# jmschrei/blueberry

Measured on AMD Instinct MI355X. Metric: Gpair-updates/s per stress iteration, N=50k, higher is better.
Workload: dtype f32

## Files before the change

blueberry_amd/csrc/bb_solver_kernels.h:

```cpp
#pragma once

#include "bb_solver_device.h"

namespace {

__device__ __forceinline__ void rsqrt_sqrt_f64(double d2, double &rinv, double &dist) {
    const double r0 = __builtin_amdgcn_rsq(d2);
    const double t = d2 * r0;
    const double e = fma(-t, r0, 1.0);
    const double q = e * fma(e, 0.375, 0.5);
    rinv = fma(r0, q, r0);
    dist = fma(t, q, t);
}
__device__ __forceinline__ double weight01_f64(double delta) {
    return __builtin_fmin(__builtin_fmax(delta * 0x1p1000, 0.0), 1.0);
}

__device__ __forceinline__ double rcp_f64(double x) {
    const double r0 = __builtin_amdgcn_rcp(x);
    const double e = fma(-x, r0, 1.0);
    return fma(r0, fma(e, e, e), r0);
}

template <int C, int OP>
__device__ __forceinline__ void pair_step(const double2 &drow, double xi, double yi, double zi,
                                          const double (&xj)[2][3], double (&gc)[2][3], double &gx,
                                          double &gy, double &gz, double &s) {
    using T = double;
    const T delta = C == 0 ? drow.x : drow.y;
    if constexpr (OP == kOpMatvec2) {
        const T a = delta * delta;
        gx += a * xj[C][0]; gy += a * xj[C][1]; gz += a * xj[C][2];
        gc[C][0] += a * xi; gc[C][1] += a * yi; gc[C][2] += a * zi;
        return;
    }
    const T dx = xi - xj[C][0], dy = yi - xj[C][1], dz = zi - xj[C][2];
    const T d2 = fma(dx, dx, fma(dy, dy, fma(dz, dz, Traits<T>::eps2())));
    T rinv, dist;
    rsqrt_sqrt_f64(d2, rinv, dist);
    if constexpr (is_weighted_op<OP>()) {
        const T m = weight01_f64(delta);
        const T res = fma(dist, m, -delta);
        const T r = rcp_f64(delta + (1.0 - m));
        const T u = res * r;
        T coef;
        if constexpr (OP == kOpStressW1) {
            s = fma(res, u, s);
            coef = u * rinv;
        } else {
            s = fma(u, u, s);
            coef = (u * r) * rinv;
        }
        gx = fma(coef, dx, gx); gy = fma(coef, dy, gy); gz = fma(coef, dz, gz);
        gc[C][0] = fma(-coef, dx, gc[C][0]);
        gc[C][1] = fma(-coef, dy, gc[C][1]);
        gc[C][2] = fma(-coef, dz, gc[C][2]);
        return;
    }
    const T res = fma(dist, weight01_f64(delta), -delta);
    s = fma(res, res, s);
    const T coef = res * rinv;
    gx = fma(coef, dx, gx); gy = fma(coef, dy, gy); gz = fma(coef, dz, gz);
    gc[C][0] = fma(-coef, dx, gc[C][0]);
    gc[C][1] = fma(-coef, dy, gc[C][1]);
    gc[C][2] = fma(-coef, dz, gc[C][2]);
}

typedef float f32x4_raw __attribute__((ext_vector_type(4)));
typedef double f64x2_raw __attribute__((ext_vector_type(2)));
template <bool NT>
__device__ __forceinline__ float4 stream_load(const float4 *p) {
    if constexpr (NT) {
        const f32x4_raw v = __builtin_nontemporal_load(reinterpret_cast<const f32x4_raw *>(p));
        return make_float4(v.x, v.y, v.z, v.w);
    } else {
        return *p;
    }
}
template <bool NT>
__device__ __forceinline__ double2 stream_load(const double2 *p) {
    if constexpr (NT) {
        const f64x2_raw v = __builtin_nontemporal_load(reinterpret_cast<const f64x2_raw *>(p));
        return make_double2(v.x, v.y);
    } else {
        return *p;
    }
}

template <typename Vec>
struct WinPtr {
    const Vec *p;
    template <bool NT>
    __device__ __forceinline__ Vec load(int k) const { return stream_load<NT>(p + k * 64); }
};

template <bool NT, int OP, typename XR, typename WIN>
__device__ __forceinline__ void process_unit_f64n(double2 (&d)[8], const XR &xrow, const WIN &next,
                                                  const double (&xj)[1][2][3], double (&gc)[1][2][3],
                                                  double &stress, __amdgpu_buffer_rsrc_t row_rsrc,
                                                  unsigned row_voff) {
    double s = 0.0;
#pragma unroll
    for (int r = 0; r < 8; ++r) {
        const double xi = xrow.get(3 * r), yi = xrow.get(3 * r + 1), zi = xrow.get(3 * r + 2);
        double gx = 0.0, gy = 0.0, gz = 0.0;
        pair_step<0, OP>(d[r], xi, yi, zi, xj[0], gc[0], gx, gy, gz, s);
        pair_step<1, OP>(d[r], xi, yi, zi, xj[0], gc[0], gx, gy, gz, s);
        d[r] = next.template load<NT>(r);
        wave_sum_hi3(gx, gy, gz);
        store_row3(row_rsrc, row_voff + r * 24u, gx, gy, gz);
        __builtin_amdgcn_sched_barrier(0);
    }
    stress += s;
}

typedef double f64x4 __attribute__((ext_vector_type(4)));

__device__ __forceinline__ double swap_sum16(double t) {
    const unsigned lo = (unsigned)__double2loint(t), hi = (unsigned)__double2hiint(t);
    const auto a = __builtin_amdgcn_permlane16_swap(lo, lo, false, false);
    const auto b = __builtin_amdgcn_permlane16_swap(hi, hi, false, false);
    return __hiloint2double((int)b[0], (int)a[0]) + __hiloint2double((int)b[1], (int)a[1]);
}
__device__ __forceinline__ double swap_sum32(double t) {
    const unsigned lo = (unsigned)__double2loint(t), hi = (unsigned)__double2hiint(t);
    const auto a = __builtin_amdgcn_permlane32_swap(lo, lo, false, false);
    const auto b = __builtin_amdgcn_permlane32_swap(hi, hi, false, false);
    return __hiloint2double((int)b[0], (int)a[0]) + __hiloint2double((int)b[1], (int)a[1]);
}

__device__ __forceinline__ float swap_add32(float a, float b) {
    const auto s = __builtin_amdgcn_permlane32_swap(__float_as_uint(a), __float_as_uint(b), false, false);
    return __uint_as_float(s[0]) + __uint_as_float(s[1]);
}
__device__ __forceinline__ float swap_add16(float a, float b) {
    const auto s = __builtin_amdgcn_permlane16_swap(__float_as_uint(a), __float_as_uint(b), false, false);
    return __uint_as_float(s[0]) + __uint_as_float(s[1]);
}
__device__ __forceinline__ float row16_sum3(float a, float b, float c) {
    float t, u, w;
    asm("s_nop 1\n\t"
        "v_add_f32_dpp %0, %3, %3 row_mirror row_mask:0xf bank_mask:0xf\n\t"
        "v_add_f32_dpp %0, %5, %5 row_mirror row_mask:0xf bank_mask:0xc\n\t"
        "v_add_f32_dpp %1, %4, %4 row_mirror row_mask:0xf bank_mask:0xf\n\t"
        "s_nop 0\n\t"
        "v_add_f32_dpp %2, %0, %0 row_half_mirror row_mask:0xf bank_mask:0xf\n\t"
        "v_add_f32_dpp %2, %1, %1 row_half_mirror row_mask:0xf bank_mask:0x2\n\t"
        "s_nop 1\n\t"
        "v_add_f32_dpp %2, %2, %2 quad_perm:[1,0,3,2] row_mask:0xf bank_mask:0xf\n\t"
        "s_nop 1\n\t"
        "v_add_f32_dpp %2, %2, %2 quad_perm:[2,3,0,1] row_mask:0xf bank_mask:0xf"
        : "=&v"(t), "=v"(u), "=v"(w)
        : "v"(a), "v"(b), "v"(c));
    return w;
}
template <int R>
__device__ __forceinline__ void row_sums_step(const float (&g)[12], float (&h)[6], float (&m)[3]) {
    if constexpr (R == 0) h[0] = swap_add32(g[0], g[1]);
    if constexpr (R == 1) {
        h[1] = swap_add32(g[2], g[3]); h[2] = swap_add32(g[4], g[5]);
        m[0] = swap_add16(h[0], h[1]);
    }
    if constexpr (R == 2) { h[3] = swap_add32(g[6], g[7]); m[1] = swap_add16(h[2], h[3]); }
    if constexpr (R == 3) {
        h[4] = swap_add32(g[8], g[9]); h[5] = swap_add32(g[10], g[11]);
        m[2] = swap_add16(h[4], h[5]);
    }
}
__device__ __forceinline__ int swap_rowsum_slot(int lane) {
    const int row = lane >> 4, bank = (lane >> 2) & 3;
    return 4 * (bank < 3 ? bank : 2) + ((row & 1) << 1) + (row >> 1);
}
__device__ __forceinline__ bool swap_rowsum_stores(int lane) { return (lane & 3) == 0 && (lane & 12) != 12; }

template <bool NT, int OP, typename XR, typename WIN>
__device__ __forceinline__ void process_unit_f64w(double2 (&d)[8], const XR &xrow,
                                                  const WIN &next,
                                                  const double (&xj)[4][2][3], double (&gc)[4][2][3],
                                                  const double (&sel)[6], double &stress,
                                                  __amdgpu_buffer_rsrc_t row_rsrc, unsigned row_voff,
                                                  int stage_idx) {
    extern __shared__ __attribute__((aligned(16))) float row_lds[];
    double s = 0.0;
    f64x4 acc = {0.0, 0.0, 0.0, 0.0};
#pragma unroll
    for (int r = 0; r < 2; ++r) {
        const double xi = xrow.get(3 * r), yi = xrow.get(3 * r + 1), zi = xrow.get(3 * r + 2);
        double gx = 0.0, gy = 0.0, gz = 0.0;
#pragma unroll
        for (int k = 0; k < 4; ++k) {
            pair_step<0, OP>(d[r * 4 + k], xi, yi, zi, xj[k], gc[k], gx, gy, gz, s);
            pair_step<1, OP>(d[r * 4 + k], xi, yi, zi, xj[k], gc[k], gx, gy, gz, s);
            d[r * 4 + k] = next.template load<NT>(r * 4 + k);
        }
        acc = __builtin_amdgcn_mfma_f64_16x16x4f64(gx, sel[3 * r + 0], acc, 0, 0, 0);
        acc = __builtin_amdgcn_mfma_f64_16x16x4f64(gy, sel[3 * r + 1], acc, 0, 0, 0);
        acc = __builtin_amdgcn_mfma_f64_16x16x4f64(gz, sel[3 * r + 2], acc, 0, 0, 0);
    }
    double t = (acc.x + acc.y) + (acc.z + acc.w);
    t = swap_sum16(t);
    t = swap_sum32(t);
    *reinterpret_cast<double *>(row_lds + stage_idx) = t;
    const u32x2 bits = {(unsigned)__double2loint(t), (unsigned)__double2hiint(t)};
    __builtin_amdgcn_raw_buffer_store_b64(bits, row_rsrc, row_voff, 0, 0);
    stress += s;
}

typedef float f32x2 __attribute__((ext_vector_type(2)));

struct StripF32 {
    f32x2 x[2][2][3];
    f32x2 g[2][2][3];
};

__device__ __forceinline__ f32x2 weight01(f32x2 delta) {
    f32x2 w;
    const f32x2 big = {0x1p100f, 0x1p100f};
    asm("v_pk_mul_f32 %0, %1, %2 clamp" : "=v"(w) : "v"(delta), "v"(big));
    return w;
}

template <int K, int H, bool FIRST, int OP, bool MASK = true>
__device__ __forceinline__ void pair_step2(f32x2 delta, f32x2 xi, f32x2 yi, f32x2 zi, StripF32 &st,
                                           f32x2 &rx, f32x2 &ry, f32x2 &rz, f32x2 &s2) {
    static_assert(MASK || OP == kOpStress, "only the plain stress sweep has a mask-free form");
    if constexpr (OP == kOpMatvec2) {
        const f32x2 a = delta * delta;
        if constexpr (FIRST) {
            rx = a * st.x[K][H][0]; ry = a * st.x[K][H][1]; rz = a * st.x[K][H][2];
        } else {
            rx += a * st.x[K][H][0]; ry += a * st.x[K][H][1]; rz += a * st.x[K][H][2];
        }
        st.g[K][H][0] += a * xi;
        st.g[K][H][1] += a * yi;
        st.g[K][H][2] += a * zi;
        return;
    }
    const f32x2 eps2 = {1e-30f, 1e-30f};
    const f32x2 dx = xi - st.x[K][H][0], dy = yi - st.x[K][H][1], dz = zi - st.x[K][H][2];
    const f32x2 d2 = dx * dx + (dy * dy + (dz * dz + eps2));
    f32x2 rinv;
    rinv.x = __builtin_amdgcn_rsqf(d2.x);
    rinv.y = __builtin_amdgcn_rsqf(d2.y);
    if constexpr (is_weighted_op<OP>()) {
        const f32x2 res = (d2 * rinv - delta) * weight01(delta);
        f32x2 a = delta;
        if constexpr (OP == kOpStressW2) a = delta * delta;
        f32x2 w;
        w.x = __builtin_amdgcn_rcpf(__builtin_fmaxf(a.x, 0x1p-126f));
        w.y = __builtin_amdgcn_rcpf(__builtin_fmaxf(a.y, 0x1p-126f));
        const f32x2 t = res * w;
        s2 += res * t;
        const f32x2 coef = t * rinv;
        if constexpr (FIRST) {
            rx = coef * dx; ry = coef * dy; rz = coef * dz;
        } else {
            rx += coef * dx; ry += coef * dy; rz += coef * dz;
        }
        st.g[K][H][0] -= coef * dx;
        st.g[K][H][1] -= coef * dy;
        st.g[K][H][2] -= coef * dz;
        return;
    }
    f32x2 res = d2 * rinv - delta;
    if constexpr (MASK) res *= weight01(delta);
    s2 += res * res;
    const f32x2 coef = res * rinv;
    if constexpr (FIRST) {
        rx = coef * dx; ry = coef * dy; rz = coef * dz;
    } else {
        rx += coef * dx; ry += coef * dy; rz += coef * dz;
    }
    st.g[K][H][0] -= coef * dx;
    st.g[K][H][1] -= coef * dy;
    st.g[K][H][2] -= coef * dz;
}

template <bool ROW3>
__device__ __forceinline__ void pk24_decode(float &word, unsigned base) {
    if constexpr (ROW3) {
        asm volatile("v_add_u32 %0, %0, %1" : "+v"(word) : "s"(base));
    } else {
        asm volatile("v_mad_u32_u24 %0, %0, 1, %1" : "+v"(word) : "s"(base));
    }
}
template <bool ROW3>
__device__ __forceinline__ void pk24_decode(float4 &w, unsigned base) {
    pk24_decode<ROW3>(w.x, base); pk24_decode<ROW3>(w.y, base);
    pk24_decode<ROW3>(w.z, base); pk24_decode<ROW3>(w.w, base);
}
__device__ __forceinline__ void pk24_decode_to(float &dst, float src, unsigned base) {
    asm volatile("v_mad_u32_u24 %0, %1, 1, %2" : "=v"(dst) : "v"(src), "s"(base));
}
__device__ __forceinline__ void pk24_decode_to(float4 &dst, const float4 &src, unsigned base) {
    pk24_decode_to(dst.x, src.x, base); pk24_decode_to(dst.y, src.y, base);
    pk24_decode_to(dst.z, src.z, base); pk24_decode_to(dst.w, src.w, base);
}
constexpr unsigned kPk24SelPair = 0x0c0c0703u;
constexpr unsigned kPk24SelThird = 0x0c070100u;
__device__ __forceinline__ float pk24_tops(float hi, float lo, unsigned sel) {
    float v;
    asm volatile("v_perm_b32 %0, %1, %2, %3" : "=v"(v) : "v"(hi), "v"(lo), "s"(sel));
    return v;
}
__device__ __forceinline__ float4 pk24_tops(float4 hi, float4 lo, unsigned sel) {
    return make_float4(pk24_tops(hi.x, lo.x, sel), pk24_tops(hi.y, lo.y, sel),
                       pk24_tops(hi.z, lo.z, sel), pk24_tops(hi.w, lo.w, sel));
}

template <bool NT, int OP, bool PK = false, typename WIN>
__device__ __forceinline__ void process_unit_f32(float4 (&d)[8], const float (&xrow)[12],
                                                 const WIN &next, StripF32 &st,
                                                 double &stress, __amdgpu_buffer_rsrc_t row_rsrc,
                                                 unsigned row_voff, int stage_idx,
                                                 unsigned base = 0u) {
    extern __shared__ __attribute__((aligned(16))) float row_lds[];
    f32x2 s2 = {0.f, 0.f};
    float g[12], h[6], m[3];
    auto row = [&](auto rc) __attribute__((always_inline)) {
        constexpr int r = decltype(rc)::value;
        const float xs = xrow[3 * r], ys = xrow[3 * r + 1], zs = xrow[3 * r + 2];
        const f32x2 xi = {xs, xs}, yi = {ys, ys}, zi = {zs, zs};
        f32x2 rx, ry, rz;
        if constexpr (PK) {
            constexpr int A = r < 3 ? 2 * r : 6, B = r == 0 ? 1 : (r == 1 ? 2 : (r == 2 ? 5 : 7));
            if constexpr (r == 0) d[6] = pk24_tops(d[1], d[0], kPk24SelPair);
            if constexpr (r == 1) d[6] = pk24_tops(d[2], d[6], kPk24SelThird);
            if constexpr (r == 2) {
                d[7] = pk24_tops(d[3], pk24_tops(d[5], d[4], kPk24SelPair), kPk24SelThird);
                d[3] = next.template load<NT>(3);
            }
            pk24_decode<r == 3>(d[A], base);
            pair_step2<0, 0, true, OP, false>(f32x2{d[A].x, d[A].y}, xi, yi, zi, st, rx, ry, rz, s2);
            pair_step2<0, 1, false, OP, false>(f32x2{d[A].z, d[A].w}, xi, yi, zi, st, rx, ry, rz, s2);
            if constexpr (r == 0) d[0] = next.template load<NT>(0);
            if constexpr (r == 2) d[4] = next.template load<NT>(4);
            if constexpr (r == 1) pk24_decode_to(d[2], d[3], base);
            else pk24_decode<r == 3>(d[B], base);
            pair_step2<1, 0, false, OP, false>(f32x2{d[B].x, d[B].y}, xi, yi, zi, st, rx, ry, rz, s2);
            pair_step2<1, 1, false, OP, false>(f32x2{d[B].z, d[B].w}, xi, yi, zi, st, rx, ry, rz, s2);
            if constexpr (r == 0) d[1] = next.template load<NT>(1);
            if constexpr (r == 1) d[2] = next.template load<NT>(2);
            if constexpr (r == 2) d[5] = next.template load<NT>(5);
            g[3 * r] = rx.x + rx.y; g[3 * r + 1] = ry.x + ry.y; g[3 * r + 2] = rz.x + rz.y;
            row_sums_step<r>(g, h, m);
            return;
        }
        pair_step2<0, 0, true, OP>(f32x2{d[2 * r].x, d[2 * r].y}, xi, yi, zi, st, rx, ry, rz, s2);
        pair_step2<0, 1, false, OP>(f32x2{d[2 * r].z, d[2 * r].w}, xi, yi, zi, st, rx, ry, rz, s2);
        d[2 * r] = next.template load<NT>(2 * r);
        pair_step2<1, 0, false, OP>(f32x2{d[2 * r + 1].x, d[2 * r + 1].y}, xi, yi, zi, st, rx, ry, rz, s2);
        pair_step2<1, 1, false, OP>(f32x2{d[2 * r + 1].z, d[2 * r + 1].w}, xi, yi, zi, st, rx, ry, rz, s2);
        d[2 * r + 1] = next.template load<NT>(2 * r + 1);
        g[3 * r] = rx.x + rx.y; g[3 * r + 1] = ry.x + ry.y; g[3 * r + 2] = rz.x + rz.y;
        row_sums_step<r>(g, h, m);
    };
    row(std::integral_constant<int, 0>{});
    row(std::integral_constant<int, 1>{});
    row(std::integral_constant<int, 2>{});
    row(std::integral_constant<int, 3>{});
    const float keep = row16_sum3(m[0], m[1], m[2]);
    row_lds[stage_idx] = keep;
    __builtin_amdgcn_raw_buffer_store_b32(__float_as_uint(keep), row_rsrc, row_voff, 0, 0);
    stress += (double)(s2.x + s2.y);
}

__device__ __forceinline__ void load_strip(StripF32 &st, const float *__restrict__ X, int j0,
                                           int lane) {
#pragma unroll
    for (int k = 0; k < 2; ++k) {
        const float4 *p = reinterpret_cast<const float4 *>(
            X + ((int64_t)j0 + k * 256 + (int64_t)lane * 4) * 3);
        const float4 a = p[0], b = p[1], c = p[2];
        st.x[k][0][0] = f32x2{a.x, a.w}; st.x[k][0][1] = f32x2{a.y, b.x};
        st.x[k][0][2] = f32x2{a.z, b.y};
        st.x[k][1][0] = f32x2{b.z, c.y}; st.x[k][1][1] = f32x2{b.w, c.z};
        st.x[k][1][2] = f32x2{c.x, c.w};
#pragma unroll
        for (int h = 0; h < 2; ++h)
#pragma unroll
            for (int c3 = 0; c3 < 3; ++c3) st.g[k][h][c3] = f32x2{0.f, 0.f};
    }
}

__device__ __forceinline__ void store_strip(const StripF32 &st, float *__restrict__ slot,
                                            int lane) {
#pragma unroll
    for (int k = 0; k < 2; ++k) {
        float4 *p = reinterpret_cast<float4 *>(slot + (k * 256 + (int64_t)lane * 4) * 3);
        const auto &g = st.g[k];
        p[0] = make_float4(g[0][0].x, g[0][1].x, g[0][2].x, g[0][0].y);
        p[1] = make_float4(g[0][1].y, g[0][2].y, g[1][0].x, g[1][1].x);
        p[2] = make_float4(g[1][2].x, g[1][0].y, g[1][1].y, g[1][2].y);
    }
}

template <typename T>
__device__ __forceinline__ const typename Traits<T>::Vec *unit_ptr(const T *__restrict__ units,
                                                                   int64_t ul, int lane) {
    using Vec = typename Traits<T>::Vec;
    return reinterpret_cast<const Vec *>(units) + ul * 512 + lane;
}

template <typename T, bool W>
__device__ __forceinline__ T load_xrow(const T *__restrict__ X, int i0, int lane) {
    return X[(int64_t)i0 * 3 + (lane < 3 * Lay<T, W>::RPU ? lane : 0)];
}

template <int LPR>
struct StripF64 {
    double xj[LPR][2][3], gc[LPR][2][3];
};
template <int LPR>
__device__ __forceinline__ void load_strip(StripF64<LPR> &st, const double *__restrict__ X, int j0,
                                           int lane) {
#pragma unroll
    for (int k = 0; k < LPR; ++k) {
        const double2 *p =
            reinterpret_cast<const double2 *>(X + ((int64_t)j0 + k * 128 + (int64_t)lane * 2) * 3);
        const double2 a = p[0], b = p[1], c = p[2];
        st.xj[k][0][0] = a.x; st.xj[k][0][1] = a.y; st.xj[k][0][2] = b.x;
        st.xj[k][1][0] = b.y; st.xj[k][1][1] = c.x; st.xj[k][1][2] = c.y;
    }
#pragma unroll
    for (int k = 0; k < LPR; ++k)
#pragma unroll
        for (int c = 0; c < 2; ++c) st.gc[k][c][0] = st.gc[k][c][1] = st.gc[k][c][2] = 0.0;
}
template <int LPR>
__device__ __forceinline__ void store_strip(const StripF64<LPR> &st, double *__restrict__ slot,
                                            int lane) {
#pragma unroll
    for (int k = 0; k < LPR; ++k) {
        double2 *p = reinterpret_cast<double2 *>(slot + ((int64_t)k * 128 + (int64_t)lane * 2) * 3);
        const auto &g = st.gc[k];
        p[0] = make_double2(g[0][0], g[0][1]);
        p[1] = make_double2(g[0][2], g[1][0]);
        p[2] = make_double2(g[1][1], g[1][2]);
    }
}
__device__ __forceinline__ int64_t pk24_word_offset(const int4 &e) { return (int64_t)(e.z & 0x7fffffff) * 64; }
__device__ __forceinline__ int64_t pk24_word_offset(const int2 &) { return 0; }
__device__ __forceinline__ bool pk24_packed(const int4 &e) { return e.z < 0; }
__device__ __forceinline__ bool pk24_packed(const int2 &) { return false; }
__device__ __forceinline__ unsigned pk24_base(const int4 &e) { return (unsigned)e.w; }
__device__ __forceinline__ unsigned pk24_base(const int2 &) { return 0u; }
__device__ __forceinline__ bool pk24_packed_body(const int4 &e) { return e.z < 0 && e.w != 0; }
__device__ __forceinline__ bool pk24_packed_body(const int2 &) { return false; }

template <typename T, bool W, bool NT, int OP, int WPB>
__global__ __launch_bounds__(64 * WPB, (Lay<T, W>::MIN_WG)) void stress_grad_kernel(
    const T *__restrict__ units, const T *__restrict__ X, const int2 *__restrict__ udesc,
    int chunk_q, int chunk_r, const int2 *__restrict__ wave_slots, T *__restrict__ rowpart,
    T *__restrict__ colpart, double *__restrict__ stresspart, int cap_units, int lds_wave_floats,
    int dense_u0, double *__restrict__ stress_slot) {
    constexpr bool PK = sizeof(T) == 0;
#include "bb_sweep_body.inc"
}

template <typename T, bool W, bool NT, int OP, int WPB>
__global__ __launch_bounds__(64 * WPB, (WPB == 8 ? 2 : 1)) void stream24_grad_kernel(
    const T *__restrict__ units, const T *__restrict__ X, const int2 *__restrict__ udesc,
    int chunk_q, int chunk_r, const int2 *__restrict__ wave_slots, T *__restrict__ rowpart,
    T *__restrict__ colpart, double *__restrict__ stresspart, int cap_units, int lds_wave_floats,
    int dense_u0, double *__restrict__ stress_slot) {
    static_assert(sizeof(T) == 4 && W, "the 24-bit stream is fp32 only");
    constexpr bool PK = sizeof(T) == 4;
#include "bb_sweep_body.inc"
}

template <typename T>
struct ReduceParams {
    const T *__restrict__ part;
    const double *__restrict__ stresspart;
    T *__restrict__ X;
    T *__restrict__ V;
    T mu;
    T scale;
    T *__restrict__ exch;
    const PeerTable<T> *__restrict__ peer;
    unsigned *__restrict__ peer_counter;
    const PeerState *peer_state;
    unsigned long long seq;
    int n_peers;
    double *__restrict__ stress_out;
    int64_t n_pad;
    int n_waves;
    int mode;
    T lr;
    const double *__restrict__ stress_slot;
    int n_slots;
    const T *__restrict__ bin_scale;
    const unsigned *__restrict__ peer_mask;
    int rank;
    const int *__restrict__ map_ptr;
    const int *__restrict__ map_idx;
    int n_maps;
};

template <typename T>
__device__ __forceinline__ double stress_share(const ReduceParams<T> &p, int m, int tid, int stride) {
    double s = 0.0;
    if (p.n_maps <= 1) {
        for (int i = tid; i < p.n_waves; i += stride) s += p.stresspart[i];
        for (int i = tid; i < p.n_slots; i += stride) s += p.stress_slot[i];
    } else {
        for (int i = p.map_ptr[m] + tid; i < p.map_ptr[m + 1]; i += stride) {
            const int idx = p.map_idx[i];
            s += idx < p.n_waves ? p.stresspart[idx] : p.stress_slot[idx - p.n_waves];
        }
    }
    return s;
}

constexpr int kRedWG = 128;

template <int S, typename T>
__device__ __forceinline__ T list_slice_sum(const T *__restrict__ part, const int64_t *__restrict__ lists,
                                            int list_stride, int b, int sl, int e) {
    const int lps = list_stride / S;
    const int64_t *list = lists + (int64_t)b * list_stride + (int64_t)sl * lps;
    T acc = T(0);
    for (int k = 0; k < lps; k += 16) {
        T v[16];
#pragma unroll
        for (int q = 0; q < 16; ++q) v[q] = part[list[k + q] + e];
#pragma unroll
        for (int q = 0; q < 16; ++q) acc += v[q];
    }
    return acc;
}
template <int S, typename T>
__device__ __forceinline__ T slices_total(const T (&meet)[S][kRedWG], int el) {
    T tot = meet[0][el];
#pragma unroll
    for (int q = 1; q < S; ++q) tot += meet[q][el];
    return tot;
}
template <typename T>
__device__ __forceinline__ T gradient_element(const ReduceParams<T> &p, int64_t o, T tot) {
    return p.bin_scale ? p.bin_scale[o / 3] * (p.scale * tot) : p.scale * tot;
}

template <typename T, bool W, int S>
__global__ __launch_bounds__(128 * S) void reduce_sliced_kernel(ReduceParams<T> p,
                                                                const int64_t *__restrict__ lists,
                                                                int list_stride) {
    constexpr int CH = 3 * Lay<T, W>::VW;
    static_assert(CH % kRedWG == 0, "3*vw is a multiple of 128");
    const int tid = threadIdx.x;
    const int el = tid & (kRedWG - 1);
    const int sl = __builtin_amdgcn_readfirstlane(tid >> 7);
    const int b = blockIdx.x;
    const int e = (int)blockIdx.y * kRedWG + el;
    __shared__ __attribute__((aligned(16))) T meet[S][kRedWG];
    const bool peer_live =
        p.mode != kReducePeer ||
        __hip_atomic_load(&p.peer_state->status, __ATOMIC_RELAXED, __HIP_MEMORY_SCOPE_AGENT) == 0;
    if (p.mode != kReduceStressOnly) {
        const int64_t o = (int64_t)b * CH + e;
        T xo = T(0), vo = T(0);
        if (p.mode == kReduceApply && sl == 0) { xo = p.X[o]; vo = p.V[o]; }
        meet[sl][el] = list_slice_sum<S>(p.part, lists, list_stride, b, sl, e);
        __syncthreads();
        if (sl == 0) {
            const T g = gradient_element(p, o, slices_total(meet, el));
            if (p.mode == kReduceApply) {
                momentum_step(p.X, p.V, o, xo, vo, p.mu, p.lr, g);
            } else if (p.mode == kReducePeer) {
                meet[0][el] = g;
            } else {
                p.exch[o] = g;
            }
        }
        if (p.mode == kReducePeer && peer_live) {
            typedef T vec_t __attribute__((ext_vector_type(16 / sizeof(T))));
            constexpr int NV = kRedWG * (int)sizeof(T) / 16;
            __syncthreads();
            if (tid < NV && (p.peer_mask == nullptr || (p.peer_mask[b] >> p.rank & 1u))) {
                const vec_t val = ((const vec_t *)meet[0])[tid];
                for (int q = 0; q < p.n_peers; ++q)
                    ((vec_t *)(p.peer->dst[q] + (int64_t)b * CH + (int64_t)blockIdx.y * kRedWG))[tid] = val;
            }
        }
    }
    if (b < (p.n_maps > 1 ? p.n_maps : 1) && blockIdx.y == 0) {
        __shared__ double sh[128 * S];
        sh[tid] = stress_share(p, b, tid, 128 * S);
        __syncthreads();
        lds_tree_fold(sh, tid, 128 * S);
        if (tid == 0) {
            const double Sx = sh[0];
            T hi, lo;
            split_hi_lo(Sx, hi, lo);
            if (p.mode == kReduceExchange) {
                p.exch[3 * p.n_pad] = hi;
                p.exch[3 * p.n_pad + 1] = lo;
            } else if (p.mode == kReducePeer) {
                for (int q = 0; q < (peer_live ? p.n_peers : 0); ++q) {
                    p.peer->dst[q][3 * p.n_pad] = hi;
                    p.peer->dst[q][3 * p.n_pad + 1] = lo;
                }
            } else {
                p.stress_out[b] = Sx;
            }
        }
    }
    if (p.mode == kReducePeer && peer_live) {
        __shared__ int last;
        asm volatile("s_waitcnt vmcnt(0)" ::: "memory");
        __syncthreads();
        if (tid == 0) {
            __builtin_amdgcn_fence(__ATOMIC_RELEASE, "");
            asm volatile("s_waitcnt vmcnt(0)" ::: "memory");
            unsigned *mine = p.peer_counter + 32 * (b + 1);
            last = 0;
            if (atomicAdd(mine, 1u) == gridDim.y - 1) {
                atomicExch(mine, 0u);
                last = atomicAdd(p.peer_counter, 1u) == gridDim.x - 1;
            }
        }
        __syncthreads();
        if (last) {
            if (tid == 0) atomicExch(p.peer_counter, 0u);
            __builtin_amdgcn_fence(__ATOMIC_ACQUIRE, "agent");
            if (tid < p.n_peers)
                __hip_atomic_store(p.peer->flag[tid], p.seq, __ATOMIC_RELEASE,
                                   __HIP_MEMORY_SCOPE_SYSTEM);
        }
    }
}

__device__ __forceinline__ bool peer_word_empty(float v) { return __float_as_uint(v) == 0xffffffffu; }
__device__ __forceinline__ bool peer_word_empty(double v) { return __double_as_longlong(v) == -1ll; }
__device__ __forceinline__ float peer_empty_word(float) { return __uint_as_float(0xffffffffu); }
__device__ __forceinline__ double peer_empty_word(double) { return __longlong_as_double(-1ll); }
template <typename T>
__device__ __forceinline__ T peer_sendable(T v) {
    return peer_word_empty(v) ? (T)__builtin_nanf("") : v;
}

template <typename T, int NW>
__device__ __forceinline__ bool peer_wait_sum(const T *base, bool active, int R, int64_t slot_elems,
                                              const PeerTableX<T> *xt, const unsigned long long *my_poison,
                                              PeerState *state, long long limit, T &sum, double &pair_sum,
                                              unsigned mask = ~0u) {
    const int lane = threadIdx.x & 63;
    T v[NW][kMaxPeers];
    bool ok = false;
    const long long t0 = wall_clock64();
    for (;;) {
        bool missing = false;
#pragma unroll
        for (int r = 0; r < kMaxPeers; ++r) {
            if (r < R) {
                const bool sends = (mask >> r & 1u) != 0;
#pragma unroll
                for (int w = 0; w < NW; ++w) {
// ... 726 lines not shown
```

blueberry_amd/csrc/bb_sweep_body.inc:

```
    using Vec = typename Traits<T>::Vec;
    constexpr int VW = Lay<T, W>::VW;
    constexpr bool DEFER = sizeof(T) == 4 || W;
    const int lane = threadIdx.x & 63;
    const int wib = __builtin_amdgcn_readfirstlane(threadIdx.x >> 6);
    const int wg = (int)blockIdx.x;
    const int w = wg * WPB + wib;
    const int ua = w * chunk_q + (w < chunk_r ? w : chunk_r);
    const int ub = ua + chunk_q + (w < chunk_r ? 1 : 0);
    double stress = 0.0;
    int ws_shared[WPB];
#pragma unroll
    for (int k = 0; k < WPB; ++k) ws_shared[k] = wave_slots[(int64_t)wg * WPB + k].y;
    extern __shared__ __attribute__((aligned(16))) float row_lds[];
    const int stage0 = wib * lds_wave_floats;
    int *progress = reinterpret_cast<int *>(row_lds + WPB * lds_wave_floats);
    int partner_done = 0;
    const int park_from = (ub - ua) > cap_units ? (ub - ua) - cap_units : 0;
    double sel[6];
#pragma unroll
    for (int v = 0; v < 6; ++v) sel[v] = (lane & 15) == v ? 1.0 : 0.0;

    if (ua < ub) {
        int slot = wave_slots[w].x;
        Vec d[8];
        using Strip = typename std::conditional<sizeof(T) == 4, StripF32,
                                                StripF64<Lay<T, W>::LPR>>::type;
        Strip st;
        auto strip_load = [&](int j0) __attribute__((always_inline)) { load_strip(st, X, j0, lane); };
        auto strip_store = [&](int sl) __attribute__((always_inline)) {
            store_strip(st, colpart + (int64_t)sl * (3 * VW), lane);
        };

        using Desc = typename std::conditional<PK, int4, int2>::type;
        const Desc *__restrict__ const table = reinterpret_cast<const Desc *>(udesc);
        Desc dc;
        if (dense_u0 >= 0) {
            constexpr int UPT = VW / Lay<T, W>::RPU;
            const unsigned g = (unsigned)dense_u0 + (unsigned)ua;
            const unsigned t = g / UPT, sub = g % UPT;
            unsigned J = (unsigned)((__builtin_sqrtf(8.0f * (float)t + 1.0f) - 1.0f) * 0.5f);
            while (J * (J + 1) / 2 > t) --J;
            while ((J + 1) * (J + 2) / 2 <= t) ++J;
            const unsigned I = t - J * (J + 1) / 2;
            if constexpr (PK) {
                dc = table[ua];
                dc.x = (int)(I * VW + sub * Lay<T, W>::RPU), dc.y = (int)(J * VW);
            } else {
                dc = make_int2((int)(I * VW + sub * Lay<T, W>::RPU), (int)(J * VW));
            }
        } else {
            dc = table[ua];
        }
        Desc dn = table[ua + 1 < ub ? ua + 1 : ua];
        struct XRowS {
            T v[3 * Lay<T, W>::RPU];
            __device__ __forceinline__ T get(int q) const { return v[q]; }
        };
        struct XRowV {
            T v;
            __device__ __forceinline__ T get(int q) const { return lane_value(v, q); }
        };
        using XRow = typename std::conditional<Lay<T, W>::SCALAR_XROW, XRowS, XRowV>::type;
        auto xrow_load = [&](int i0) __attribute__((always_inline)) {
            XRow x;
            if constexpr (std::is_same<XRow, XRowS>::value) {
                const T *px = X + (int64_t)i0 * 3;
#pragma unroll
                for (int q = 0; q < 3 * Lay<T, W>::RPU; ++q) x.v[q] = px[q];
            } else {
                x.v = load_xrow<T, W>(X, i0, lane);
            }
            return x;
        };
        XRow xr = xrow_load(dc.x);
        using Win = WinPtr<Vec>;
        auto window_of = [&](int u_next) __attribute__((always_inline)) {
            const bool real = u_next < ub;
            if constexpr (PK) {
                return Win{reinterpret_cast<const Vec *>(units) + pk24_word_offset(dn) +
                           (real ? lane : 0)};
            } else {
                return Win{unit_ptr<T>(units, real ? u_next : ub - 1, real ? lane : 0)};
            }
        };
        auto window_here = [&]() __attribute__((always_inline)) {
            return Win{reinterpret_cast<const Vec *>(units) + pk24_word_offset(dc) + lane};
        };
        if constexpr (PK) {
            const Win first = window_here();
#pragma unroll
            for (int r = 0; r < 6; ++r) d[r] = first.template load<NT>(r);
        } else {
            const Win first = window_of(ua);
#pragma unroll
            for (int r = 0; r < 8; ++r) d[r] = first.template load<NT>(r);
        }
        constexpr unsigned kRowBytes = 3 * Lay<T, W>::RPU * sizeof(T);
        const __amdgpu_buffer_rsrc_t row_rsrc = __builtin_amdgcn_make_buffer_rsrc(
            rowpart + (int64_t)ua * (3 * Lay<T, W>::RPU), 0, (int)((unsigned)(ub - ua) * kRowBytes),
            0x00020000);

        const int f32_sl12 = swap_rowsum_slot(lane);
        const unsigned f32_voff_lane = swap_rowsum_stores(lane) ? (unsigned)f32_sl12 * 4u : 0x40000000u;
        const int f32_lds_lane = stage0 + f32_sl12;
        auto unit_step = [&](int u, auto packed_body) __attribute__((always_inline)) {
            if constexpr (WPB == 8) {
                const int mine = u - ua;
                if (__builtin_amdgcn_readfirstlane(partner_done) > mine)
                    __builtin_amdgcn_s_setprio(1);
                else
                    __builtin_amdgcn_s_setprio(0);
                __hip_atomic_store(progress + wib, mine, __ATOMIC_RELAXED, __HIP_MEMORY_SCOPE_WORKGROUP);
                partner_done = __hip_atomic_load(progress + (wib ^ 4), __ATOMIC_RELAXED,
                                                 __HIP_MEMORY_SCOPE_WORKGROUP);
            }
            const int un = u + 1 < ub ? u + 1 : u;
            const XRow xrn = xrow_load(dn.x);
            const Desc dnn = table[un + 1 < ub ? un + 1 : un];
            const int k = u - ua;
            const bool parked = k >= park_from;
            if constexpr (sizeof(T) == 4) {
                const unsigned row_voff =
                    f32_voff_lane + (parked ? 0x40000000u : (unsigned)k * kRowBytes);
                const int stage_slot = f32_lds_lane + (parked ? k - park_from : 0) * 12;
                float xs12[12];
#pragma unroll
                for (int q = 0; q < 12; ++q) xs12[q] = xr.get(q);
                if constexpr (decltype(packed_body)::value) {
                    process_unit_f32<NT, OP, true>(d, xs12, window_of(u + 1), st, stress, row_rsrc,
                                                   row_voff, stage_slot, pk24_base(dc));
                } else {
                    process_unit_f32<NT, OP>(d, xs12, window_of(u + 1), st, stress, row_rsrc, row_voff,
                                             stage_slot);
                }
            } else if constexpr (W) {
                const bool mine = lane >= 48 && lane < 54;
                const unsigned row_voff =
                    (mine && !parked) ? (unsigned)k * kRowBytes + (unsigned)(lane - 48) * 8u
                                      : kDropOffset;
                const int stage_slot =
                    stage0 + ((mine && parked) ? (k - park_from) * 12 + (lane - 48) * 2
                                               : cap_units * 12 + 2 * (lane & 1));
                process_unit_f64w<NT, OP>(d, xr, window_of(u + 1), st.xj, st.gc, sel, stress,
                                          row_rsrc, row_voff, stage_slot);
            } else {
                const unsigned row_voff = lane == 63 ? (unsigned)k * kRowBytes : kDropOffset;
                process_unit_f64n<NT, OP>(d, xr, window_of(u + 1), st.xj, st.gc, stress,
                                          row_rsrc, row_voff);
            }
            xr = xrn;
            dc = dn;
            dn = dnn;
        };
        int u = ua;
        if constexpr (PK) {
            for (;;) {
                const int curj = dc.y;
                strip_load(curj);
                for (;;) {
                    if (pk24_packed_body(dc)) {
                        __builtin_amdgcn_s_waitcnt(0x0F70);
                        do {
                            unit_step(u, std::true_type{});
                            ++u;
                        } while (u < ub && dc.y == curj && pk24_packed_body(dc));
                    } else {
                        const bool zeros = pk24_packed(dc);
                        if (zeros) {
                            d[6] = d[7] = make_float4(0.f, 0.f, 0.f, 0.f);
                        } else {
                            const Win here = window_here();
                            d[6] = here.template load<NT>(6);
                            d[7] = here.template load<NT>(7);
                        }
                        __builtin_amdgcn_s_waitcnt(0x0F70);
                        do {
                            unit_step(u, std::false_type{});
                            ++u;
                        } while (!zeros && u < ub && dc.y == curj && !pk24_packed(dc));
                    }
                    if (u >= ub || dc.y != curj) break;
                }
                if (u >= ub) break;
                strip_store(slot);
                const double sv = wave_sum_hi(stress);
                if (lane == 63) stress_slot[slot] = sv;
                stress = 0.0;
                ++slot;
            }
        } else {
            for (;;) {
                const int curj = dc.y;
                strip_load(curj);
                __builtin_amdgcn_s_waitcnt(0x0F70);
                do {
                    unit_step(u, std::false_type{});
                    ++u;
                } while (u < ub && dc.y == curj);
                if (u >= ub) break;
                strip_store(slot);
                {
                    const double sv = wave_sum_hi(stress);
                    if (lane == 63) stress_slot[slot] = sv;
                    stress = 0.0;
                }
                ++slot;
            }
        }
        if constexpr (WPB == 8) {
            __hip_atomic_store(progress + wib, 0x7fffffff, __ATOMIC_RELAXED, __HIP_MEMORY_SCOPE_WORKGROUP);
            __builtin_amdgcn_s_setprio(0);
        }
        if constexpr (DEFER) {
            __builtin_amdgcn_fence(__ATOMIC_ACQ_REL, "wavefront");
            __builtin_amdgcn_wave_barrier();
            const int n4 = ((ub - ua) - park_from) * 3;
            float4 *dst = reinterpret_cast<float4 *>(rowpart + ((int64_t)ua + park_from) *
                                                                   (3 * Lay<T, W>::RPU));
            const int lane_q = (int)__builtin_amdgcn_mbcnt_hi(~0u, __builtin_amdgcn_mbcnt_lo(~0u, 0u));
            for (int q = lane_q; q < n4; q += 64) {
                const float *src = row_lds + stage0 + 4 * q;
                dst[q] = make_float4(src[0], src[1], src[2], src[3]);
            }
            __builtin_amdgcn_fence(__ATOMIC_ACQ_REL, "wavefront");
            __builtin_amdgcn_wave_barrier();
        }
        store_strip(st, reinterpret_cast<T *>(row_lds + stage0), lane);
    }
    __builtin_amdgcn_fence(__ATOMIC_RELEASE, "workgroup", "local");
    __builtin_amdgcn_s_barrier();
    __builtin_amdgcn_fence(__ATOMIC_ACQUIRE, "workgroup", "local");
    {
        constexpr int CH = 3 * VW, NTH = 64 * WPB;
        int k = 0;
        while (k < WPB) {
            const int sl = ws_shared[k];
            if (sl < 0) { ++k; continue; }
            int k2 = k + 1;
            while (k2 < WPB && ws_shared[k2] == sl) ++k2;
            T *dst = colpart + (int64_t)sl * CH;
#pragma unroll
            for (int j = 0; j < (CH + NTH - 1) / NTH; ++j) {
                const int e = (int)threadIdx.x + NTH * j;
                if (CH % NTH == 0 || e < CH) {
                    T acc = T(0);
                    for (int q = k; q < k2; ++q)
                        acc += reinterpret_cast<const T *>(row_lds + q * lds_wave_floats)[e];
                    dst[e] = acc;
                }
            }
            k = k2;
        }
    }

    stress = wave_sum_hi(stress);
    if (lane == 63) stresspart[w] = stress;
```

Baseline: 1827.

## Keep f32 row coordinates as SGPR pairs with packed op_sel math and in-place refresh

```diff
diff --git a/blueberry_amd/csrc/bb_solver_kernels.h b/blueberry_amd/csrc/bb_solver_kernels.h
--- a/blueberry_amd/csrc/bb_solver_kernels.h
+++ b/blueberry_amd/csrc/bb_solver_kernels.h
@@ -220,10 +220,34 @@
     return w;
 }
 
-template <int K, int H, bool FIRST, int OP, bool MASK = true>
-__device__ __forceinline__ void pair_step2(f32x2 delta, f32x2 xi, f32x2 yi, f32x2 zi, StripF32 &st,
+struct XRowS32 {
+    f32x2 p[6];
+};
+template <int HALF>
+__device__ __forceinline__ f32x2 row_minus(f32x2 pair, f32x2 xj) {
+    f32x2 d;
+    if constexpr (HALF == 0)
+        asm("v_pk_add_f32 %0, %1, %2 op_sel_hi:[0,1] neg_lo:[0,1] neg_hi:[0,1]"
+            : "=v"(d) : "s"(pair), "v"(xj));
+    else
+        asm("v_pk_add_f32 %0, %1, %2 op_sel:[1,0] op_sel_hi:[1,1] neg_lo:[0,1] neg_hi:[0,1]"
+            : "=v"(d) : "s"(pair), "v"(xj));
+    return d;
+}
+template <int HALF>
+__device__ __forceinline__ void row_fma(f32x2 &acc, f32x2 a, f32x2 pair) {
+    if constexpr (HALF == 0)
+        asm("v_pk_fma_f32 %0, %1, %2, %0 op_sel_hi:[1,0,1]" : "+v"(acc) : "v"(a), "s"(pair));
+    else
+        asm("v_pk_fma_f32 %0, %1, %2, %0 op_sel:[0,1,0] op_sel_hi:[1,1,1]"
+            : "+v"(acc) : "v"(a), "s"(pair));
+}
+
+template <int K, int H, bool FIRST, int OP, int R, bool MASK = true>
+__device__ __forceinline__ void pair_step2(f32x2 delta, const XRowS32 &xr, StripF32 &st,
                                            f32x2 &rx, f32x2 &ry, f32x2 &rz, f32x2 &s2) {
     static_assert(MASK || OP == kOpStress, "only the plain stress sweep has a mask-free form");
+    constexpr int QX = 3 * R, QY = 3 * R + 1, QZ = 3 * R + 2;
     if constexpr (OP == kOpMatvec2) {
         const f32x2 a = delta * delta;
         if constexpr (FIRST) {
@@ -231,13 +255,15 @@
         } else {
             rx += a * st.x[K][H][0]; ry += a * st.x[K][H][1]; rz += a * st.x[K][H][2];
         }
-        st.g[K][H][0] += a * xi;
-        st.g[K][H][1] += a * yi;
-        st.g[K][H][2] += a * zi;
+        row_fma<QX & 1>(st.g[K][H][0], a, xr.p[QX >> 1]);
+        row_fma<QY & 1>(st.g[K][H][1], a, xr.p[QY >> 1]);
+        row_fma<QZ & 1>(st.g[K][H][2], a, xr.p[QZ >> 1]);
         return;
     }
     const f32x2 eps2 = {1e-30f, 1e-30f};
-    const f32x2 dx = xi - st.x[K][H][0], dy = yi - st.x[K][H][1], dz = zi - st.x[K][H][2];
+    const f32x2 dx = row_minus<QX & 1>(xr.p[QX >> 1], st.x[K][H][0]),
+                dy = row_minus<QY & 1>(xr.p[QY >> 1], st.x[K][H][1]),
+                dz = row_minus<QZ & 1>(xr.p[QZ >> 1], st.x[K][H][2]);
     const f32x2 d2 = dx * dx + (dy * dy + (dz * dz + eps2));
     f32x2 rinv;
     rinv.x = __builtin_amdgcn_rsqf(d2.x);
@@ -308,9 +334,39 @@
                        pk24_tops(hi.z, lo.z, sel), pk24_tops(hi.w, lo.w, sel));
 }
 
+template <int R>
+__device__ __forceinline__ void xrow_refresh(XRowS32 &xr, const float *__restrict__ X, unsigned xnext,
+                                             float after) {
+    asm("" : "+s"(xnext) : "v"(after));
+    const f32x2 *__restrict__ px =
+        reinterpret_cast<const f32x2 *>(reinterpret_cast<const char *>(X) + xnext);
+    constexpr int P = 3 * (R >> 1);
+    if constexpr (R & 1) {
+        xr.p[P + 1] = px[P + 1];
+        xr.p[P + 2] = px[P + 2];
+    } else {
+        xr.p[P] = px[P];
+    }
+}
+
+struct WinBase32 {
+    const char *mid;
+    unsigned voff;
+    __device__ __forceinline__ WinBase32(const void *units, int64_t unit_byte, unsigned lane_off)
+        : voff(lane_off) {
+        int64_t to_mid = unit_byte + 4096;
+        asm("" : "+s"(to_mid));
+        mid = static_cast<const char *>(units) + to_mid;
+    }
+    template <bool NT>
+    __device__ __forceinline__ float4 load(int k) const {
+        return stream_load<NT>(reinterpret_cast<const float4 *>(mid + voff + (k * 1024 - 4096)));
+    }
+};
+
 template <bool NT, int OP, bool PK = false, typename WIN>
-__device__ __forceinline__ void process_unit_f32(float4 (&d)[8], const float (&xrow)[12],
-                                                 const WIN &next, StripF32 &st,
+__device__ __forceinline__ void process_unit_f32(float4 (&d)[8], XRowS32 &xrow, const float *X,
+                                                 unsigned xnext, const WIN &next, StripF32 &st,
                                                  double &stress, __amdgpu_buffer_rsrc_t row_rsrc,
                                                  unsigned row_voff, int stage_idx,
                                                  unsigned base = 0u) {
@@ -319,8 +375,6 @@
     float g[12], h[6], m[3];
     auto row = [&](auto rc) __attribute__((always_inline)) {
         constexpr int r = decltype(rc)::value;
-        const float xs = xrow[3 * r], ys = xrow[3 * r + 1], zs = xrow[3 * r + 2];
-        const f32x2 xi = {xs, xs}, yi = {ys, ys}, zi = {zs, zs};
         f32x2 rx, ry, rz;
         if constexpr (PK) {
             constexpr int A = r < 3 ? 2 * r : 6, B = r == 0 ? 1 : (r == 1 ? 2 : (r == 2 ? 5 : 7));
@@ -331,29 +385,31 @@
                 d[3] = next.template load<NT>(3);
             }
             pk24_decode<r == 3>(d[A], base);
-            pair_step2<0, 0, true, OP, false>(f32x2{d[A].x, d[A].y}, xi, yi, zi, st, rx, ry, rz, s2);
-            pair_step2<0, 1, false, OP, false>(f32x2{d[A].z, d[A].w}, xi, yi, zi, st, rx, ry, rz, s2);
+            pair_step2<0, 0, true, OP, r, false>(f32x2{d[A].x, d[A].y}, xrow, st, rx, ry, rz, s2);
+            pair_step2<0, 1, false, OP, r, false>(f32x2{d[A].z, d[A].w}, xrow, st, rx, ry, rz, s2);
             if constexpr (r == 0) d[0] = next.template load<NT>(0);
             if constexpr (r == 2) d[4] = next.template load<NT>(4);
             if constexpr (r == 1) pk24_decode_to(d[2], d[3], base);
             else pk24_decode<r == 3>(d[B], base);
-            pair_step2<1, 0, false, OP, false>(f32x2{d[B].x, d[B].y}, xi, yi, zi, st, rx, ry, rz, s2);
-            pair_step2<1, 1, false, OP, false>(f32x2{d[B].z, d[B].w}, xi, yi, zi, st, rx, ry, rz, s2);
+            pair_step2<1, 0, false, OP, r, false>(f32x2{d[B].x, d[B].y}, xrow, st, rx, ry, rz, s2);
+            pair_step2<1, 1, false, OP, r, false>(f32x2{d[B].z, d[B].w}, xrow, st, rx, ry, rz, s2);
             if constexpr (r == 0) d[1] = next.template load<NT>(1);
             if constexpr (r == 1) d[2] = next.template load<NT>(2);
             if constexpr (r == 2) d[5] = next.template load<NT>(5);
             g[3 * r] = rx.x + rx.y; g[3 * r + 1] = ry.x + ry.y; g[3 * r + 2] = rz.x + rz.y;
             row_sums_step<r>(g, h, m);
+            xrow_refresh<r>(xrow, X, xnext, g[3 * r + 2]);
             return;
         }
-        pair_step2<0, 0, true, OP>(f32x2{d[2 * r].x, d[2 * r].y}, xi, yi, zi, st, rx, ry, rz, s2);
-        pair_step2<0, 1, false, OP>(f32x2{d[2 * r].z, d[2 * r].w}, xi, yi, zi, st, rx, ry, rz, s2);
+        pair_step2<0, 0, true, OP, r>(f32x2{d[2 * r].x, d[2 * r].y}, xrow, st, rx, ry, rz, s2);
+        pair_step2<0, 1, false, OP, r>(f32x2{d[2 * r].z, d[2 * r].w}, xrow, st, rx, ry, rz, s2);
         d[2 * r] = next.template load<NT>(2 * r);
-        pair_step2<1, 0, false, OP>(f32x2{d[2 * r + 1].x, d[2 * r + 1].y}, xi, yi, zi, st, rx, ry, rz, s2);
-        pair_step2<1, 1, false, OP>(f32x2{d[2 * r + 1].z, d[2 * r + 1].w}, xi, yi, zi, st, rx, ry, rz, s2);
+        pair_step2<1, 0, false, OP, r>(f32x2{d[2 * r + 1].x, d[2 * r + 1].y}, xrow, st, rx, ry, rz, s2);
+        pair_step2<1, 1, false, OP, r>(f32x2{d[2 * r + 1].z, d[2 * r + 1].w}, xrow, st, rx, ry, rz, s2);
         d[2 * r + 1] = next.template load<NT>(2 * r + 1);
         g[3 * r] = rx.x + rx.y; g[3 * r + 1] = ry.x + ry.y; g[3 * r + 2] = rz.x + rz.y;
         row_sums_step<r>(g, h, m);
+        xrow_refresh<r>(xrow, X, xnext, g[3 * r + 2]);
     };
     row(std::integral_constant<int, 0>{});
     row(std::integral_constant<int, 1>{});
diff --git a/blueberry_amd/csrc/bb_sweep_body.inc b/blueberry_amd/csrc/bb_sweep_body.inc
--- a/blueberry_amd/csrc/bb_sweep_body.inc
+++ b/blueberry_amd/csrc/bb_sweep_body.inc
@@ -60,10 +60,19 @@
             T v;
             __device__ __forceinline__ T get(int q) const { return lane_value(v, q); }
         };
-        using XRow = typename std::conditional<Lay<T, W>::SCALAR_XROW, XRowS, XRowV>::type;
+        using XRow = typename std::conditional<
+            sizeof(T) == 4, XRowS32,
+            typename std::conditional<Lay<T, W>::SCALAR_XROW, XRowS, XRowV>::type>::type;
+        auto xrow_pairs = [&](int i0) __attribute__((always_inline)) {
+            return reinterpret_cast<const f32x2 *>(X + (int64_t)i0 * 3);
+        };
         auto xrow_load = [&](int i0) __attribute__((always_inline)) {
             XRow x;
-            if constexpr (std::is_same<XRow, XRowS>::value) {
+            if constexpr (std::is_same<XRow, XRowS32>::value) {
+                const f32x2 *px = xrow_pairs(i0);
+#pragma unroll
+                for (int q = 0; q < 6; ++q) x.p[q] = px[q];
+            } else if constexpr (std::is_same<XRow, XRowS>::value) {
                 const T *px = X + (int64_t)i0 * 3;
 #pragma unroll
                 for (int q = 0; q < 3 * Lay<T, W>::RPU; ++q) x.v[q] = px[q];
@@ -73,18 +82,26 @@
             return x;
         };
         XRow xr = xrow_load(dc.x);
-        using Win = WinPtr<Vec>;
+        using Win = typename std::conditional<sizeof(T) == 4, WinBase32, WinPtr<Vec>>::type;
+        [[maybe_unused]] const unsigned lane_off = (unsigned)lane * 16u;
         auto window_of = [&](int u_next) __attribute__((always_inline)) {
             const bool real = u_next < ub;
             if constexpr (PK) {
-                return Win{reinterpret_cast<const Vec *>(units) + pk24_word_offset(dn) +
-                           (real ? lane : 0)};
+                return Win{units, pk24_word_offset(dn) * 16,
+                           real ? lane_off : 0u};
+            } else if constexpr (sizeof(T) == 4) {
+                return Win{units, (int64_t)(real ? u_next : ub - 1) * 8192,
+                           real ? lane_off : 0u};
             } else {
                 return Win{unit_ptr<T>(units, real ? u_next : ub - 1, real ? lane : 0)};
             }
         };
         auto window_here = [&]() __attribute__((always_inline)) {
-            return Win{reinterpret_cast<const Vec *>(units) + pk24_word_offset(dc) + lane};
+            if constexpr (sizeof(T) == 4)
+                return Win{units, pk24_word_offset(dc) * 16,
+                           lane_off};
+            else
+                return Win{reinterpret_cast<const Vec *>(units) + pk24_word_offset(dc) + lane};
         };
         if constexpr (PK) {
             const Win first = window_here();
@@ -115,7 +132,8 @@
                                                  __HIP_MEMORY_SCOPE_WORKGROUP);
             }
             const int un = u + 1 < ub ? u + 1 : u;
-            const XRow xrn = xrow_load(dn.x);
+            [[maybe_unused]] XRow xrn;
+            if constexpr (sizeof(T) != 4) xrn = xrow_load(dn.x);
             const Desc dnn = table[un + 1 < ub ? un + 1 : un];
             const int k = u - ua;
             const bool parked = k >= park_from;
@@ -123,15 +141,12 @@
                 const unsigned row_voff =
                     f32_voff_lane + (parked ? 0x40000000u : (unsigned)k * kRowBytes);
                 const int stage_slot = f32_lds_lane + (parked ? k - park_from : 0) * 12;
-                float xs12[12];
-#pragma unroll
-                for (int q = 0; q < 12; ++q) xs12[q] = xr.get(q);
                 if constexpr (decltype(packed_body)::value) {
-                    process_unit_f32<NT, OP, true>(d, xs12, window_of(u + 1), st, stress, row_rsrc,
-                                                   row_voff, stage_slot, pk24_base(dc));
+                    process_unit_f32<NT, OP, true>(d, xr, X, (unsigned)dn.x * 12u, window_of(u + 1), st, stress,
+                                                   row_rsrc, row_voff, stage_slot, pk24_base(dc));
                 } else {
-                    process_unit_f32<NT, OP>(d, xs12, window_of(u + 1), st, stress, row_rsrc, row_voff,
-                                             stage_slot);
+                    process_unit_f32<NT, OP>(d, xr, X, (unsigned)dn.x * 12u, window_of(u + 1), st, stress,
+                                             row_rsrc, row_voff, stage_slot);
                 }
             } else if constexpr (W) {
                 const bool mine = lane >= 48 && lane < 54;
@@ -148,7 +163,7 @@
                 process_unit_f64n<NT, OP>(d, xr, window_of(u + 1), st.xj, st.gc, stress,
                                           row_rsrc, row_voff);
             }
-            xr = xrn;
+            if constexpr (sizeof(T) != 4) xr = xrn;
             dc = dn;
             dn = dnn;
         };
```

After: 1846, median of 6. 1.01x the previous value.
